# MiniMax-AI/VTP

Hardware: NVIDIA H100
Metric: images/sec (256x256 encode+decode+3-loss step) (higher is better)
Workload: dtype bf16

## Files before the change

vtp_b200/csrc/attention.cu:

```cuda
#include <stdlib.h>

#include "attention.h"
#include "host.h"
#include "ptx.cuh"

namespace vtp {

static constexpr int ATT_THREADS = 384;
static constexpr int MAX_PREFIX = ATT_MAX_PREFIX;
static constexpr int SQ = 0, SK = 16384, SV = SK + 32768, SBAR = SV + 32768;
static constexpr int SPCLS = SBAR + 128;
static constexpr int ATT_SMEM = SPCLS + 512 + 1024;

__device__ __forceinline__ float ex2f(float x) {
    float y;
    asm("ex2.approx.ftz.f32 %0, %1;" : "=f"(y) : "f"(x));
    return y;
}
__device__ __forceinline__ uint32_t sw128_off(int row, int col ) {
    return row * 128 + ((((col >> 3) ^ (row & 7)) << 4) | ((col & 7) << 1));
}

template <int NKT>
__global__ void __launch_bounds__(ATT_THREADS, 1) attn_fwd_kernel(const __grid_constant__ CUtensorMap tm, const AttnDev p) {
    constexpr int NK = 128 * NKT;
    extern __shared__ uint8_t smem_raw[];
    uint8_t* smem = reinterpret_cast<uint8_t*>((reinterpret_cast<uintptr_t>(smem_raw) + 1023) & ~uintptr_t(1023));
    uint64_t* bars = reinterpret_cast<uint64_t*>(smem + SBAR);
    uint64_t* bar_qk = bars + 0;
    uint64_t* bar_v = bars + 1;

    const int warp = threadIdx.x >> 5, lane = threadIdx.x & 31;
    const int qt = blockIdx.x, h = blockIdx.y, b = p.pack ? blockIdx.z * p.pack : blockIdx.z;
    const int D = p.D, T = p.T, prefix = p.prefix, HW = p.HW;
    const long seq_row0 = (long)b * T;
    const int kvrows = NK;

    if (threadIdx.x == 0) {
        tma_prefetch_desc(&tm);
        mbar_init(bar_qk, 1), mbar_init(bar_v, 1);
        fence_barrier_init();
    }
    __syncthreads();

    if (warp < 8) {
        setmaxnreg_inc<200>();
        const int wg = warp >> 2, tw = threadIdx.x & 127, c4 = lane & 3;
        int rr[2], qpos[2], qtok[2], pseq[2], kmin[2], kmax[2];
        bool row_valid[2];
#pragma unroll
        for (int i = 0; i < 2; ++i) {
            rr[i] = 64 * wg + 16 * (tw >> 5) + (lane >> 2) + 8 * i;
            qpos[i] = 128 * qt + rr[i];
            qtok[i] = prefix + qpos[i];
            pseq[i] = p.pack ? rr[i] / T : 0;
            row_valid[i] = p.pack ? (pseq[i] < p.pack && b + pseq[i] < p.B) : (qpos[i] < HW);
            kmin[i] = p.pack ? (row_valid[i] ? pseq[i] * T : 0) : 0;
            kmax[i] = p.pack ? (row_valid[i] ? kmin[i] + T : 0) : (p.causal ? min(HW, qpos[i] + 1) : HW);
        }
        mbar_wait(bar_qk, 0);
        float s[NK / 2];
        {
            const uint32_t qa = smem_u32(smem + SQ) + wg * 8192, ka = smem_u32(smem + SK);
            wgmma_fence();
#pragma unroll
            for (int j = 0; j < 4; ++j) {
                const uint64_t ad = wgmma_desc_sw128(qa + j * 32, 0, 1024), bd = wgmma_desc_sw128(ka + j * 32, 0, 1024);
                if constexpr (NKT == 2) wgmma_m64n256_ss<0, 0>(s, ad, bd, j > 0);
                else wgmma_m64n128_ss<0, 0>(s, ad, bd, j > 0);
            }
            wgmma_commit();
        }
        float s_pre[2][MAX_PREFIX];
#pragma unroll
        for (int j = 0; j < MAX_PREFIX; ++j) {
            float acc0 = 0.f, acc1 = 0.f;
            if (j < prefix) {
                const uint4* kp = reinterpret_cast<const uint4*>(p.qkv + (seq_row0 + j) * 3 * D + D + h * 64 + 16 * c4);
#pragma unroll
                for (int c = 0; c < 2; ++c) {
                    const uint4 w = __ldg(kp + c);
                    const uint4 q0 = *reinterpret_cast<const uint4*>(smem + SQ + sw128_off(rr[0], 16 * c4 + 8 * c));
                    const uint4 q1 = *reinterpret_cast<const uint4*>(smem + SQ + sw128_off(rr[1], 16 * c4 + 8 * c));
                    const uint32_t kw[4] = {w.x, w.y, w.z, w.w}, qw0[4] = {q0.x, q0.y, q0.z, q0.w}, qw1[4] = {q1.x, q1.y, q1.z, q1.w};
#pragma unroll
                    for (int e = 0; e < 4; ++e) {
                        acc0 += bf16_lo(qw0[e]) * bf16_lo(kw[e]) + bf16_hi(qw0[e]) * bf16_hi(kw[e]);
                        acc1 += bf16_lo(qw1[e]) * bf16_lo(kw[e]) + bf16_hi(qw1[e]) * bf16_hi(kw[e]);
                    }
                }
            }
            acc0 += __shfl_xor_sync(0xffffffffu, acc0, 1), acc1 += __shfl_xor_sync(0xffffffffu, acc1, 1);
            acc0 += __shfl_xor_sync(0xffffffffu, acc0, 2), acc1 += __shfl_xor_sync(0xffffffffu, acc1, 2);
            s_pre[0][j] = (j < prefix && (!p.causal || j <= qtok[0])) ? acc0 : -INFINITY;
            s_pre[1][j] = (j < prefix && (!p.causal || j <= qtok[1])) ? acc1 : -INFINITY;
        }
        wgmma_wait<0>();
        fence_regs(s);
        float m[2], msc[2], l[2];
#pragma unroll
        for (int i = 0; i < 2; ++i) {
            m[i] = -INFINITY;
#pragma unroll
            for (int j = 0; j < MAX_PREFIX; ++j) m[i] = fmaxf(m[i], s_pre[i][j]);
        }
#pragma unroll
        for (int jn = 0; jn < NK / 8; ++jn)
#pragma unroll
            for (int i = 0; i < 2; ++i)
#pragma unroll
                for (int c = 0; c < 2; ++c) {
                    const int key = 8 * jn + 2 * c4 + c;
                    if (key >= kmin[i] && key < kmax[i]) m[i] = fmaxf(m[i], s[4 * jn + 2 * i + c]);
                }
        float p_pre[2][MAX_PREFIX];
#pragma unroll
        for (int i = 0; i < 2; ++i) {
            m[i] = fmaxf(m[i], __shfl_xor_sync(0xffffffffu, m[i], 1));
            m[i] = fmaxf(m[i], __shfl_xor_sync(0xffffffffu, m[i], 2));
            msc[i] = (m[i] == -INFINITY) ? 0.f : m[i] * p.scale_log2;
            l[i] = 0.f;
#pragma unroll
            for (int j = 0; j < MAX_PREFIX; ++j) {
                p_pre[i][j] = (s_pre[i][j] == -INFINITY) ? 0.f : ex2f(s_pre[i][j] * p.scale_log2 - msc[i]);
                if (c4 == 0) l[i] += p_pre[i][j];
                p_pre[i][j] = bf16_round(p_pre[i][j]);
            }
        }
#pragma unroll
        for (int jn = 0; jn < NK / 8; ++jn)
#pragma unroll
            for (int i = 0; i < 2; ++i)
#pragma unroll
                for (int c = 0; c < 2; ++c) {
                    const int key = 8 * jn + 2 * c4 + c;
                    float& v = s[4 * jn + 2 * i + c];
                    v = (key >= kmin[i] && key < kmax[i]) ? ex2f(v * p.scale_log2 - msc[i]) : 0.f;
                    l[i] += v;
                }
        mbar_wait(bar_v, 0);
        float o[32];
        {
            const uint32_t va = smem_u32(smem + SV);
            wgmma_fence();
#pragma unroll
            for (int kk = 0; kk < NK / 16; ++kk) {
                const uint32_t a[4] = {pack_bf16x2(s[8 * kk], s[8 * kk + 1]), pack_bf16x2(s[8 * kk + 2], s[8 * kk + 3]),
                                       pack_bf16x2(s[8 * kk + 4], s[8 * kk + 5]), pack_bf16x2(s[8 * kk + 6], s[8 * kk + 7])};
                wgmma_m64n64_rs<1>(o, a, wgmma_desc_sw128(va + kk * 2048, 8192, 1024), kk > 0);
            }
            wgmma_commit();
            wgmma_wait<0>();
            fence_regs(o);
        }
#pragma unroll
        for (int i = 0; i < 2; ++i) {
            l[i] += __shfl_xor_sync(0xffffffffu, l[i], 1);
            l[i] += __shfl_xor_sync(0xffffffffu, l[i], 2);
        }
#pragma unroll
        for (int j = 0; j < MAX_PREFIX; ++j) {
            if (j < prefix) {
                const __nv_bfloat16* vp = p.qkv + (seq_row0 + j) * 3 * D + 2 * D + h * 64 + 2 * c4;
#pragma unroll
                for (int jn = 0; jn < 8; ++jn) {
                    const uint32_t w = __ldg(reinterpret_cast<const uint32_t*>(vp + 8 * jn));
#pragma unroll
                    for (int i = 0; i < 2; ++i)
                        o[4 * jn + 2 * i] += p_pre[i][j] * bf16_lo(w), o[4 * jn + 2 * i + 1] += p_pre[i][j] * bf16_hi(w);
                }
            }
        }
#pragma unroll
        for (int i = 0; i < 2; ++i) {
            if (!row_valid[i]) continue;
            const float inv = 1.f / l[i];
            __nv_bfloat16* op = p.out + (seq_row0 + qtok[i]) * D + h * 64 + 2 * c4;
#pragma unroll
            for (int jn = 0; jn < 8; ++jn)
                *reinterpret_cast<uint32_t*>(op + 8 * jn) = pack_bf16x2(o[4 * jn + 2 * i] * inv, o[4 * jn + 2 * i + 1] * inv);
            if (p.lse && c4 == 0) {
                if (p.pack) p.lse[((long)(b + pseq[i]) * p.H + h) * T + (rr[i] - pseq[i] * T)] = m[i] * p.scale + logf(l[i]);
                else p.lse[((long)b * p.H + h) * T + qtok[i]] = m[i] * p.scale + logf(l[i]);
            }
        }
    } else {
        setmaxnreg_dec<104>();
        if (warp != 8) return;
        if (lane == 0) {
            const int row_q = (int)seq_row0 + prefix + 128 * qt;
            const int row_k = (int)seq_row0 + prefix;
            mbar_expect_tx(bar_qk, 16384 + 16384 * NKT);
            tma_load_2d(smem + SQ, &tm, bar_qk, h * 64, row_q);
            for (int i = 0; i < NKT; ++i) tma_load_2d(smem + SK + i * 16384, &tm, bar_qk, D + h * 64, row_k + 128 * i);
            mbar_expect_tx(bar_v, 16384 * NKT);
            for (int i = 0; i < NKT; ++i) tma_load_2d(smem + SV + i * 16384, &tm, bar_v, 2 * D + h * 64, row_k + 128 * i);
        }
        if (qt == 0 && prefix > 0) {
            mbar_wait(bar_qk, 0);
            mbar_wait(bar_v, 0);
            for (int j = 0; j < prefix; ++j) {
                float qf[64];
                {
                    const uint4* qp = reinterpret_cast<const uint4*>(p.qkv + (seq_row0 + j) * 3 * D + h * 64);
#pragma unroll
                    for (int c = 0; c < 8; ++c) {
                        const uint4 w = __ldg(qp + c);
                        qf[c * 8 + 0] = bf16_lo(w.x), qf[c * 8 + 1] = bf16_hi(w.x), qf[c * 8 + 2] = bf16_lo(w.y);
                        qf[c * 8 + 3] = bf16_hi(w.y), qf[c * 8 + 4] = bf16_lo(w.z), qf[c * 8 + 5] = bf16_hi(w.z);
                        qf[c * 8 + 6] = bf16_lo(w.w), qf[c * 8 + 7] = bf16_hi(w.w);
                    }
                }
                auto dot_row = [&](const uint4* kp, bool from_smem, int row) {
                    float acc = 0.f;
#pragma unroll
                    for (int c = 0; c < 8; ++c) {
                        const uint4 w = from_smem ? *reinterpret_cast<const uint4*>(smem + SK + sw128_off(row, c * 8))
                                                  : __ldg(kp + c);
                        acc += qf[c * 8 + 0] * bf16_lo(w.x) + qf[c * 8 + 1] * bf16_hi(w.x) + qf[c * 8 + 2] * bf16_lo(w.y) +
                               qf[c * 8 + 3] * bf16_hi(w.y) + qf[c * 8 + 4] * bf16_lo(w.z) + qf[c * 8 + 5] * bf16_hi(w.z) +
                               qf[c * 8 + 6] * bf16_lo(w.w) + qf[c * 8 + 7] * bf16_hi(w.w);
                    }
                    return acc;
                };
                float sp[MAX_PREFIX], s[8];
                float m = -INFINITY;
#pragma unroll
                for (int t = 0; t < MAX_PREFIX; ++t) {
                    sp[t] = -INFINITY;
                    if (t < prefix && (!p.causal || t <= j))
                        sp[t] = dot_row(reinterpret_cast<const uint4*>(p.qkv + (seq_row0 + t) * 3 * D + D + h * 64), false, 0);
                    m = fmaxf(m, sp[t]);
                }
#pragma unroll
                for (int i = 0; i < 8; ++i) {
                    const int kk = lane + 32 * i;
                    s[i] = -INFINITY;
                    if (kk < HW && kk < kvrows && (!p.causal || prefix + kk <= j)) s[i] = dot_row(nullptr, true, kk);
                    m = fmaxf(m, s[i]);
                }
                m = warp_max(m);
                const float msc = m * p.scale_log2;
                float l = 0.f;
                __nv_bfloat16* pcls = reinterpret_cast<__nv_bfloat16*>(smem + SPCLS);
                __syncwarp();
#pragma unroll
                for (int i = 0; i < 8; ++i) {
                    const float e = (s[i] == -INFINITY) ? 0.f : ex2f(s[i] * p.scale_log2 - msc);
                    l += e;
                    pcls[lane + 32 * i] = __float2bfloat16_rn(e);
                }
                l = warp_sum(l);
                __syncwarp();
                float a0 = 0.f, a1 = 0.f, c0 = 0.f, c1 = 0.f;
#pragma unroll
                for (int t = 0; t < MAX_PREFIX; ++t) {
                    if (t < prefix && sp[t] != -INFINITY) {
                        const float pe = ex2f(sp[t] * p.scale_log2 - msc);
                        l += pe;
                        const uint32_t w = __ldg(reinterpret_cast<const uint32_t*>(p.qkv + (seq_row0 + t) * 3 * D + 2 * D + h * 64) + lane);
                        a0 += bf16_round(pe) * bf16_lo(w), a1 += bf16_round(pe) * bf16_hi(w);
                    }
                }
                const int kend = min(HW, kvrows);
                for (int k8 = 0; k8 < kend; k8 += 8) {
                    const uint4 pw = *reinterpret_cast<const uint4*>(pcls + k8);
                    const uint32_t pr[4] = {pw.x, pw.y, pw.z, pw.w};
#pragma unroll
                    for (int u = 0; u < 8; ++u) {
                        const float pk = (u & 1) ? bf16_hi(pr[u >> 1]) : bf16_lo(pr[u >> 1]);
                        const uint32_t w = *reinterpret_cast<const uint32_t*>(smem + SV + sw128_off(k8 + u, 2 * lane));
                        if (u & 1) c0 += pk * bf16_lo(w), c1 += pk * bf16_hi(w);
                        else a0 += pk * bf16_lo(w), a1 += pk * bf16_hi(w);
                    }
                }
                a0 += c0, a1 += c1;
                const float inv = 1.f / l;
                *reinterpret_cast<uint32_t*>(p.out + (seq_row0 + j) * D + h * 64 + 2 * lane) = pack_bf16x2(a0 * inv, a1 * inv);
                if (p.lse && lane == 0) p.lse[((long)b * p.H + h) * T + j] = m * p.scale + logf(l);
            }
        }
    }
}


__global__ void attn_fwd_f32_kernel(const float* __restrict__ qkv, float* __restrict__ out, int T, int H, int causal,
                                    float scale) {
    extern __shared__ float sm[];
    const int D = H * 64, h = blockIdx.x, b = blockIdx.y;
    float* Ks = sm;
    float* Vs = Ks + (long)T * 65;
    float* Ps = Vs + (long)T * 64;
    const float* base = qkv + (long)b * T * 3 * D;
    for (int i = threadIdx.x; i < T * 64; i += blockDim.x) {
        const int t = i >> 6, d = i & 63;
        Ks[t * 65 + d] = base[(long)t * 3 * D + D + h * 64 + d];
        Vs[t * 64 + d] = base[(long)t * 3 * D + 2 * D + h * 64 + d];
    }
    __syncthreads();
    const int warp = threadIdx.x >> 5, lane = threadIdx.x & 31, nw = blockDim.x >> 5;
    float* pw = Ps + (long)warp * T;
    for (int q = warp; q < T; q += nw) {
        const float* qp = base + (long)q * 3 * D + h * 64;
        float qf[64];
#pragma unroll
        for (int d = 0; d < 64; ++d) qf[d] = qp[d];
        const int kend = causal ? q + 1 : T;
        float m = -INFINITY;
        for (int k = lane; k < kend; k += 32) {
            float acc = 0.f;
#pragma unroll
            for (int d = 0; d < 64; ++d) acc += qf[d] * Ks[k * 65 + d];
            acc *= scale;
            pw[k] = acc;
            m = fmaxf(m, acc);
        }
        m = warp_max(m);
        float l = 0.f;
        for (int k = lane; k < kend; k += 32) {
            const float e = expf(pw[k] - m);
            pw[k] = e;
            l += e;
        }
        l = warp_sum(l);
        __syncwarp();
        float a0 = 0.f, a1 = 0.f;
        for (int k = 0; k < kend; ++k) {
            const float pk = pw[k];
            a0 += pk * Vs[k * 64 + lane], a1 += pk * Vs[k * 64 + 32 + lane];
        }
        float* op = out + ((long)b * T + q) * D + h * 64;
        op[lane] = a0 / l, op[32 + lane] = a1 / l;
        __syncwarp();
    }
}

}

using namespace vtp;

extern "C" int vtp_attention_fwd(const void* qkv, void* out, float* lse, int B, int T, int H, int prefix, int causal,
                                 vtp_stream_t st) {
    VTP_CHECK_ARG(qkv && out && B > 0 && T > 0 && H > 0, "attention_fwd: bad args");
    VTP_CHECK_ARG(prefix >= 0 && prefix <= MAX_PREFIX && prefix < T, "attention_fwd: prefix must be in [0,%d]", MAX_PREFIX);
    const int HW = T - prefix;
    VTP_CHECK_ARG(HW <= 256 || !causal, "attention_fwd: causal attention over %d > 256 non-prefix tokens is not supported",
                  HW);
    VTP_CHECK_ARG(B <= 65535 && H <= 65535, "attention_fwd: grid too large");
    const int D = H * 64;
    AttnDev p;
    p.qkv = (const __nv_bfloat16*)qkv, p.out = (__nv_bfloat16*)out, p.lse = lse;
    p.B = B, p.T = T, p.H = H, p.D = D, p.prefix = prefix, p.HW = HW, p.causal = causal;
    p.nkt = HW > 128 ? 2 : 1;
    p.scale = 0.125f;
    p.scale_log2 = 0.125f * 1.4426950408889634f;
    p.pack = 0;
    if (!causal && T <= 64 && B > 1 && getenv("VTP_ATTN_NO_PACK") == nullptr) {
        p.pack = 128 / T;
        p.prefix = 0, p.HW = T, p.nkt = 1;
    }
    CUtensorMap tm;
    uint64_t dims[2] = {(uint64_t)3 * D, (uint64_t)B * T}, strides[1] = {(uint64_t)3 * D * 2};
    uint32_t box[2] = {64, 128};
    int rc = make_tmap_bf16(&tm, qkv, 2, dims, strides, box);
    if (rc) return rc;
    if (HW > 256) return attn_fwd_long(tm, p, (cudaStream_t)st);
    static bool configured = false;
    if (!configured) {
        VTP_CUDA(cudaFuncSetAttribute(attn_fwd_kernel<1>, cudaFuncAttributeMaxDynamicSharedMemorySize, ATT_SMEM));
        VTP_CUDA(cudaFuncSetAttribute(attn_fwd_kernel<2>, cudaFuncAttributeMaxDynamicSharedMemorySize, ATT_SMEM));
        configured = true;
    }
    dim3 grid(p.pack ? 1 : ceil_div(HW, 128), H, p.pack ? ceil_div(B, p.pack) : B);
    if (p.nkt == 2) attn_fwd_kernel<2><<<grid, ATT_THREADS, ATT_SMEM, (cudaStream_t)st>>>(tm, p);
    else attn_fwd_kernel<1><<<grid, ATT_THREADS, ATT_SMEM, (cudaStream_t)st>>>(tm, p);
    VTP_LAUNCH_CHECK();
    return VTP_OK;
}

extern "C" int vtp_attention_fwd_f32(const float* qkv, float* out, int B, int T, int H, int causal, vtp_stream_t st) {
    VTP_CHECK_ARG(qkv && out && B > 0 && T > 0 && H > 0 && B <= 65535, "attention_fwd_f32: bad args");
    const int nw = 8;
    const size_t smem = ((size_t)T * 65 + (size_t)T * 64 + (size_t)nw * T) * sizeof(float);
    if (smem > 220 * 1024) {
        VTP_CHECK_ARG(!causal, "attention_fwd_f32: causal attention over T=%d (beyond the smem-resident kernel) is not "
                               "supported", T);
        return attn_fwd_f32_tiled(qkv, out, B, T, H, (cudaStream_t)st);
    }
    static size_t configured = 0;
    if (smem > configured) {
        VTP_CUDA(cudaFuncSetAttribute(attn_fwd_f32_kernel, cudaFuncAttributeMaxDynamicSharedMemorySize, (int)smem));
        configured = smem;
    }
    attn_fwd_f32_kernel<<<dim3(H, B), nw * 32, smem, (cudaStream_t)st>>>(qkv, out, T, H, causal, 0.125f);
    VTP_LAUNCH_CHECK();
    return VTP_OK;
}
```

Measured before the change: 704.4.

## Make short-sequence attention forward persistent with double-buffered TMA and parallel prefix warps

Result: faster. 719.0, median of 6 (+2.1%).

```diff
diff --git a/vtp_b200/csrc/attention.cu b/vtp_b200/csrc/attention.cu
--- a/vtp_b200/csrc/attention.cu
+++ b/vtp_b200/csrc/attention.cu
@@ -8,9 +8,17 @@
 
 static constexpr int ATT_THREADS = 384;
 static constexpr int MAX_PREFIX = ATT_MAX_PREFIX;
-static constexpr int SQ = 0, SK = 16384, SV = SK + 32768, SBAR = SV + 32768;
-static constexpr int SPCLS = SBAR + 128;
-static constexpr int ATT_SMEM = SPCLS + 512 + 1024;
+static constexpr int PREFIX_WARPS = 3;
+static constexpr int CONSUMER_REGS = 200, WG2_REGS = 104;
+template <int NKT>
+struct FwdSmem {
+    static constexpr int TILE = 16384 * NKT;
+    static constexpr int SLOT = 3 * TILE;
+    static constexpr int BAR = 2 * SLOT;
+    static constexpr int PCLS = BAR + 64;
+    static constexpr int QCLS = PCLS + PREFIX_WARPS * 512;
+    static constexpr int BYTES = QCLS + PREFIX_WARPS * 128 + 1024;
+};
 
 __device__ __forceinline__ float ex2f(float x) {
     float y;
@@ -21,268 +29,300 @@
     return row * 128 + ((((col >> 3) ^ (row & 7)) << 4) | ((col & 7) << 1));
 }
 
+template <int NKT, bool DENSE>
+__device__ __forceinline__ void fwd_block(const AttnDev& p, const uint8_t* sl, int blk, int h, int b, long seq_row0) {
+    constexpr int NK = 128 * NKT;
+    constexpr int TILE = FwdSmem<NKT>::TILE;
+    const int lane = threadIdx.x & 31, tw = threadIdx.x & 127, c4 = lane & 3;
+    const int D = p.D, T = p.T, prefix = p.prefix, HW = p.HW;
+    int rr[2], qtok[2], pseq[2], kmin[2], kmax[2];
+    bool row_valid[2];
+#pragma unroll
+    for (int i = 0; i < 2; ++i) {
+        rr[i] = 64 * blk + 16 * (tw >> 5) + (lane >> 2) + 8 * i;
+        qtok[i] = prefix + rr[i];
+        pseq[i] = p.pack ? rr[i] / T : 0;
+        row_valid[i] = p.pack ? (pseq[i] < p.pack && b + pseq[i] < p.B) : (rr[i] < HW);
+        kmin[i] = p.pack ? (row_valid[i] ? pseq[i] * T : 0) : 0;
+        kmax[i] = p.pack ? (row_valid[i] ? kmin[i] + T : 0) : (p.causal ? min(HW, rr[i] + 1) : HW);
+    }
+    float s[NK / 2];
+    {
+        const uint32_t qa = smem_u32(sl) + blk * 8192, ka = smem_u32(sl + TILE);
+        wgmma_fence();
+#pragma unroll
+        for (int j = 0; j < 4; ++j) {
+            const uint64_t ad = wgmma_desc_sw128(qa + j * 32, 0, 1024), bd = wgmma_desc_sw128(ka + j * 32, 0, 1024);
+            if constexpr (NKT == 2) wgmma_m64n256_ss<0, 0>(s, ad, bd, j > 0);
+            else wgmma_m64n128_ss<0, 0>(s, ad, bd, j > 0);
+        }
+        wgmma_commit();
+    }
+    float s_pre[2][MAX_PREFIX];
+#pragma unroll
+    for (int j = 0; j < MAX_PREFIX; ++j) {
+        float acc0 = 0.f, acc1 = 0.f;
+        if (j < prefix) {
+            const uint4* kp = reinterpret_cast<const uint4*>(p.qkv + (seq_row0 + j) * 3 * D + D + h * 64 + 16 * c4);
+#pragma unroll
+            for (int c = 0; c < 2; ++c) {
+                const uint4 w = __ldg(kp + c);
+                const uint4 q0 = *reinterpret_cast<const uint4*>(sl + sw128_off(rr[0], 16 * c4 + 8 * c));
+                const uint4 q1 = *reinterpret_cast<const uint4*>(sl + sw128_off(rr[1], 16 * c4 + 8 * c));
+                const uint32_t kw[4] = {w.x, w.y, w.z, w.w}, qw0[4] = {q0.x, q0.y, q0.z, q0.w}, qw1[4] = {q1.x, q1.y, q1.z, q1.w};
+#pragma unroll
+                for (int e = 0; e < 4; ++e) {
+                    acc0 += bf16_lo(qw0[e]) * bf16_lo(kw[e]) + bf16_hi(qw0[e]) * bf16_hi(kw[e]);
+                    acc1 += bf16_lo(qw1[e]) * bf16_lo(kw[e]) + bf16_hi(qw1[e]) * bf16_hi(kw[e]);
+                }
+            }
+        }
+        acc0 += __shfl_xor_sync(0xffffffffu, acc0, 1), acc1 += __shfl_xor_sync(0xffffffffu, acc1, 1);
+        acc0 += __shfl_xor_sync(0xffffffffu, acc0, 2), acc1 += __shfl_xor_sync(0xffffffffu, acc1, 2);
+        s_pre[0][j] = (j < prefix && (!p.causal || j <= qtok[0])) ? acc0 : -INFINITY;
+        s_pre[1][j] = (j < prefix && (!p.causal || j <= qtok[1])) ? acc1 : -INFINITY;
+    }
+    wgmma_wait<0>();
+    fence_regs(s);
+    float m[2], msc[2], l[2];
+#pragma unroll
+    for (int i = 0; i < 2; ++i) {
+        m[i] = -INFINITY;
+#pragma unroll
+        for (int j = 0; j < MAX_PREFIX; ++j) m[i] = fmaxf(m[i], s_pre[i][j]);
+    }
+#pragma unroll
+    for (int jn = 0; jn < NK / 8; ++jn)
+#pragma unroll
+        for (int i = 0; i < 2; ++i)
+#pragma unroll
+            for (int c = 0; c < 2; ++c) {
+                const int key = 8 * jn + 2 * c4 + c;
+                if (DENSE || (key >= kmin[i] && key < kmax[i])) m[i] = fmaxf(m[i], s[4 * jn + 2 * i + c]);
+            }
+    float p_pre[2][MAX_PREFIX];
+#pragma unroll
+    for (int i = 0; i < 2; ++i) {
+        m[i] = fmaxf(m[i], __shfl_xor_sync(0xffffffffu, m[i], 1));
+        m[i] = fmaxf(m[i], __shfl_xor_sync(0xffffffffu, m[i], 2));
+        msc[i] = (m[i] == -INFINITY) ? 0.f : m[i] * p.scale_log2;
+        l[i] = 0.f;
+#pragma unroll
+        for (int j = 0; j < MAX_PREFIX; ++j) {
+            p_pre[i][j] = (s_pre[i][j] == -INFINITY) ? 0.f : ex2f(s_pre[i][j] * p.scale_log2 - msc[i]);
+            if (c4 == 0) l[i] += p_pre[i][j];
+            p_pre[i][j] = bf16_round(p_pre[i][j]);
+        }
+    }
+    uint32_t a[NK / 4];
+#pragma unroll
+    for (int jn = 0; jn < NK / 8; ++jn) {
+        float v[4];
+#pragma unroll
+        for (int i = 0; i < 2; ++i)
+#pragma unroll
+            for (int c = 0; c < 2; ++c) {
+                const int key = 8 * jn + 2 * c4 + c;
+                const float x = s[4 * jn + 2 * i + c];
+                v[2 * i + c] = (DENSE || (key >= kmin[i] && key < kmax[i])) ? ex2f(x * p.scale_log2 - msc[i]) : 0.f;
+                l[i] += v[2 * i + c];
+            }
+        a[2 * jn] = pack_bf16x2(v[0], v[1]), a[2 * jn + 1] = pack_bf16x2(v[2], v[3]);
+    }
+    float o[32];
+    {
+        const uint32_t va = smem_u32(sl + 2 * TILE);
+        wgmma_fence();
+#pragma unroll
+        for (int kk = 0; kk < NK / 16; ++kk) {
+            const uint32_t ak[4] = {a[4 * kk], a[4 * kk + 1], a[4 * kk + 2], a[4 * kk + 3]};
+            wgmma_m64n64_rs<1>(o, ak, wgmma_desc_sw128(va + kk * 2048, 8192, 1024), kk > 0);
+        }
+        wgmma_commit();
+        wgmma_wait<0>();
+        fence_regs(o);
+    }
+#pragma unroll
+    for (int i = 0; i < 2; ++i) {
+        l[i] += __shfl_xor_sync(0xffffffffu, l[i], 1);
+        l[i] += __shfl_xor_sync(0xffffffffu, l[i], 2);
+    }
+#pragma unroll
+    for (int j = 0; j < MAX_PREFIX; ++j) {
+        if (j < prefix) {
+            const __nv_bfloat16* vp = p.qkv + (seq_row0 + j) * 3 * D + 2 * D + h * 64 + 2 * c4;
+#pragma unroll
+            for (int jn = 0; jn < 8; ++jn) {
+                const uint32_t w = __ldg(reinterpret_cast<const uint32_t*>(vp + 8 * jn));
+#pragma unroll
+                for (int i = 0; i < 2; ++i)
+                    o[4 * jn + 2 * i] += p_pre[i][j] * bf16_lo(w), o[4 * jn + 2 * i + 1] += p_pre[i][j] * bf16_hi(w);
+            }
+        }
+    }
+#pragma unroll
+    for (int i = 0; i < 2; ++i) {
+        if (!row_valid[i]) continue;
+        const float inv = 1.f / l[i];
+        __nv_bfloat16* op = p.out + (seq_row0 + qtok[i]) * D + h * 64 + 2 * c4;
+#pragma unroll
+        for (int jn = 0; jn < 8; ++jn)
+            *reinterpret_cast<uint32_t*>(op + 8 * jn) = pack_bf16x2(o[4 * jn + 2 * i] * inv, o[4 * jn + 2 * i + 1] * inv);
+        if (p.lse && c4 == 0) {
+            if (p.pack) p.lse[((long)(b + pseq[i]) * p.H + h) * T + (rr[i] - pseq[i] * T)] = m[i] * p.scale + logf(l[i]);
+            else p.lse[((long)b * p.H + h) * T + qtok[i]] = m[i] * p.scale + logf(l[i]);
+        }
+    }
+}
+
 template <int NKT>
-__global__ void __launch_bounds__(ATT_THREADS, 1) attn_fwd_kernel(const __grid_constant__ CUtensorMap tm, const AttnDev p) {
+__device__ __forceinline__ void fwd_prefix_row(const AttnDev& p, const uint8_t* sl, uint4* qs, __nv_bfloat16* pcls, int j,
+                                               int h, int b, long seq_row0) {
     constexpr int NK = 128 * NKT;
+    constexpr int TILE = FwdSmem<NKT>::TILE;
+    const int lane = threadIdx.x & 31;
+    const int D = p.D, T = p.T, prefix = p.prefix, HW = p.HW;
+    const uint8_t* sk = sl + TILE;
+    const uint8_t* sv = sl + 2 * TILE;
+    __syncwarp();
+    if (lane < 8) qs[lane] = __ldg(reinterpret_cast<const uint4*>(p.qkv + (seq_row0 + j) * 3 * D + h * 64) + lane);
+    __syncwarp();
+    auto dot_row = [&](const uint4* kp, bool from_smem, int row) {
+        float acc = 0.f;
+#pragma unroll 1
+        for (int c = 0; c < 8; ++c) {
+            const uint4 w = from_smem ? *reinterpret_cast<const uint4*>(sk + sw128_off(row, c * 8)) : __ldg(kp + c);
+            const uint4 q = qs[c];
+            acc += bf16_lo(q.x) * bf16_lo(w.x) + bf16_hi(q.x) * bf16_hi(w.x) + bf16_lo(q.y) * bf16_lo(w.y) +
+                   bf16_hi(q.y) * bf16_hi(w.y) + bf16_lo(q.z) * bf16_lo(w.z) + bf16_hi(q.z) * bf16_hi(w.z) +
+                   bf16_lo(q.w) * bf16_lo(w.w) + bf16_hi(q.w) * bf16_hi(w.w);
+        }
+        return acc;
+    };
+    float sp[MAX_PREFIX], s[8];
+    float m = -INFINITY;
+#pragma unroll
+    for (int t = 0; t < MAX_PREFIX; ++t) {
+        sp[t] = -INFINITY;
+        if (t < prefix && (!p.causal || t <= j))
+            sp[t] = dot_row(reinterpret_cast<const uint4*>(p.qkv + (seq_row0 + t) * 3 * D + D + h * 64), false, 0);
+        m = fmaxf(m, sp[t]);
+    }
+#pragma unroll
+    for (int i = 0; i < 8; ++i) {
+        const int kk = lane + 32 * i;
+        s[i] = -INFINITY;
+        if (kk < HW && kk < NK && (!p.causal || prefix + kk <= j)) s[i] = dot_row(nullptr, true, kk);
+        m = fmaxf(m, s[i]);
+    }
+    m = warp_max(m);
+    const float msc = m * p.scale_log2;
+    float l = 0.f;
+    __syncwarp();
+#pragma unroll
+    for (int i = 0; i < 8; ++i) {
+        const float e = (s[i] == -INFINITY) ? 0.f : ex2f(s[i] * p.scale_log2 - msc);
+        l += e;
+        pcls[lane + 32 * i] = __float2bfloat16_rn(e);
+    }
+    l = warp_sum(l);
+    __syncwarp();
+    float a0 = 0.f, a1 = 0.f, c0 = 0.f, c1 = 0.f;
+#pragma unroll
+    for (int t = 0; t < MAX_PREFIX; ++t) {
+        if (t < prefix && sp[t] != -INFINITY) {
+            const float pe = ex2f(sp[t] * p.scale_log2 - msc);
+            l += pe;
+            const uint32_t w = __ldg(reinterpret_cast<const uint32_t*>(p.qkv + (seq_row0 + t) * 3 * D + 2 * D + h * 64) + lane);
+            a0 += bf16_round(pe) * bf16_lo(w), a1 += bf16_round(pe) * bf16_hi(w);
+        }
+    }
+    const int kend = min(HW, NK);
+    for (int k8 = 0; k8 < kend; k8 += 8) {
+        const uint4 pw = *reinterpret_cast<const uint4*>(pcls + k8);
+        const uint32_t pr[4] = {pw.x, pw.y, pw.z, pw.w};
+#pragma unroll
+        for (int u = 0; u < 8; ++u) {
+            const float pk = (u & 1) ? bf16_hi(pr[u >> 1]) : bf16_lo(pr[u >> 1]);
+            const uint32_t w = *reinterpret_cast<const uint32_t*>(sv + sw128_off(k8 + u, 2 * lane));
+            if (u & 1) c0 += pk * bf16_lo(w), c1 += pk * bf16_hi(w);
+            else a0 += pk * bf16_lo(w), a1 += pk * bf16_hi(w);
+        }
+    }
+    a0 += c0, a1 += c1;
+    const float inv = 1.f / l;
+    *reinterpret_cast<uint32_t*>(p.out + (seq_row0 + j) * D + h * 64 + 2 * lane) = pack_bf16x2(a0 * inv, a1 * inv);
+    if (p.lse && lane == 0) p.lse[((long)b * p.H + h) * T + j] = m * p.scale + logf(l);
+}
+
+template <int NKT, bool DENSE>
+__global__ void __launch_bounds__(ATT_THREADS, 1)
+    attn_fwd_persistent_kernel(const __grid_constant__ CUtensorMap tm, const AttnDev p) {
+    using L = FwdSmem<NKT>;
     extern __shared__ uint8_t smem_raw[];
     uint8_t* smem = reinterpret_cast<uint8_t*>((reinterpret_cast<uintptr_t>(smem_raw) + 1023) & ~uintptr_t(1023));
-    uint64_t* bars = reinterpret_cast<uint64_t*>(smem + SBAR);
-    uint64_t* bar_qk = bars + 0;
-    uint64_t* bar_v = bars + 1;
+    uint64_t* full = reinterpret_cast<uint64_t*>(smem + L::BAR);
+    uint64_t* empty = full + 2;
 
     const int warp = threadIdx.x >> 5, lane = threadIdx.x & 31;
-    const int qt = blockIdx.x, h = blockIdx.y, b = p.pack ? blockIdx.z * p.pack : blockIdx.z;
-    const int D = p.D, T = p.T, prefix = p.prefix, HW = p.HW;
-    const long seq_row0 = (long)b * T;
-    const int kvrows = NK;
+    const int H = p.H, T = p.T, prefix = p.prefix;
+    const int items = (p.pack ? (p.B + p.pack - 1) / p.pack : p.B) * H;
+    const int prefix_warps = min(prefix, PREFIX_WARPS);
 
     if (threadIdx.x == 0) {
         tma_prefetch_desc(&tm);
-        mbar_init(bar_qk, 1), mbar_init(bar_v, 1);
+        for (int s = 0; s < 2; ++s) mbar_init(full + s, 1), mbar_init(empty + s, 8 + prefix_warps);
         fence_barrier_init();
     }
     __syncthreads();
 
     if (warp < 8) {
-        setmaxnreg_inc<200>();
-        const int wg = warp >> 2, tw = threadIdx.x & 127, c4 = lane & 3;
-        int rr[2], qpos[2], qtok[2], pseq[2], kmin[2], kmax[2];
-        bool row_valid[2];
-#pragma unroll
-        for (int i = 0; i < 2; ++i) {
-            rr[i] = 64 * wg + 16 * (tw >> 5) + (lane >> 2) + 8 * i;
-            qpos[i] = 128 * qt + rr[i];
-            qtok[i] = prefix + qpos[i];
-            pseq[i] = p.pack ? rr[i] / T : 0;
-            row_valid[i] = p.pack ? (pseq[i] < p.pack && b + pseq[i] < p.B) : (qpos[i] < HW);
-            kmin[i] = p.pack ? (row_valid[i] ? pseq[i] * T : 0) : 0;
-            kmax[i] = p.pack ? (row_valid[i] ? kmin[i] + T : 0) : (p.causal ? min(HW, qpos[i] + 1) : HW);
-        }
-        mbar_wait(bar_qk, 0);
-        float s[NK / 2];
-        {
-            const uint32_t qa = smem_u32(smem + SQ) + wg * 8192, ka = smem_u32(smem + SK);
-            wgmma_fence();
-#pragma unroll
-            for (int j = 0; j < 4; ++j) {
-                const uint64_t ad = wgmma_desc_sw128(qa + j * 32, 0, 1024), bd = wgmma_desc_sw128(ka + j * 32, 0, 1024);
-                if constexpr (NKT == 2) wgmma_m64n256_ss<0, 0>(s, ad, bd, j > 0);
-                else wgmma_m64n128_ss<0, 0>(s, ad, bd, j > 0);
-            }
-            wgmma_commit();
-        }
-        float s_pre[2][MAX_PREFIX];
-#pragma unroll
-        for (int j = 0; j < MAX_PREFIX; ++j) {
-            float acc0 = 0.f, acc1 = 0.f;
-            if (j < prefix) {
-                const uint4* kp = reinterpret_cast<const uint4*>(p.qkv + (seq_row0 + j) * 3 * D + D + h * 64 + 16 * c4);
-#pragma unroll
-                for (int c = 0; c < 2; ++c) {
-                    const uint4 w = __ldg(kp + c);
-                    const uint4 q0 = *reinterpret_cast<const uint4*>(smem + SQ + sw128_off(rr[0], 16 * c4 + 8 * c));
-                    const uint4 q1 = *reinterpret_cast<const uint4*>(smem + SQ + sw128_off(rr[1], 16 * c4 + 8 * c));
-                    const uint32_t kw[4] = {w.x, w.y, w.z, w.w}, qw0[4] = {q0.x, q0.y, q0.z, q0.w}, qw1[4] = {q1.x, q1.y, q1.z, q1.w};
-#pragma unroll
-                    for (int e = 0; e < 4; ++e) {
-                        acc0 += bf16_lo(qw0[e]) * bf16_lo(kw[e]) + bf16_hi(qw0[e]) * bf16_hi(kw[e]);
-                        acc1 += bf16_lo(qw1[e]) * bf16_lo(kw[e]) + bf16_hi(qw1[e]) * bf16_hi(kw[e]);
-                    }
+        setmaxnreg_inc<CONSUMER_REGS>();
+        const int wg = __shfl_sync(0xffffffffu, warp >> 2, 0);
+        int it = 0;
+        for (int item = blockIdx.x; item < items; item += gridDim.x, ++it) {
+            const int slot = it & 1, h = item % H, sq = item / H;
+            const int b = p.pack ? sq * p.pack : sq;
+            const int nrows = p.pack ? min(p.pack, p.B - b) * T : p.HW;
+            const uint8_t* sl = smem + slot * L::SLOT;
+            mbar_wait(full + slot, (it >> 1) & 1);
+#pragma unroll 1
+            for (int blk = wg; 64 * blk < nrows; blk += 2) fwd_block<NKT, DENSE>(p, sl, blk, h, b, (long)b * T);
+            __syncwarp();
+            if (lane == 0) mbar_arrive(empty + slot);
+        }
+    } else {
+        setmaxnreg_dec<WG2_REGS>();
+        if (warp == 8) {
+            if (lane != 0) return;
+            int it = 0;
+            for (int item = blockIdx.x; item < items; item += gridDim.x, ++it) {
+                const int slot = it & 1, h = item % H, sq = item / H;
+                const int row0 = (p.pack ? sq * p.pack : sq) * T + prefix;
+                uint8_t* sl = smem + slot * L::SLOT;
+                if (it >= 2) mbar_wait(empty + slot, ((it >> 1) - 1) & 1);
+                mbar_expect_tx(full + slot, 3 * L::TILE);
+                for (int i = 0; i < NKT; ++i) {
+                    tma_load_2d(sl + i * 16384, &tm, full + slot, h * 64, row0 + 128 * i);
+                    tma_load_2d(sl + L::TILE + i * 16384, &tm, full + slot, p.D + h * 64, row0 + 128 * i);
+                    tma_load_2d(sl + 2 * L::TILE + i * 16384, &tm, full + slot, 2 * p.D + h * 64, row0 + 128 * i);
                 }
             }
-            acc0 += __shfl_xor_sync(0xffffffffu, acc0, 1), acc1 += __shfl_xor_sync(0xffffffffu, acc1, 1);
-            acc0 += __shfl_xor_sync(0xffffffffu, acc0, 2), acc1 += __shfl_xor_sync(0xffffffffu, acc1, 2);
-            s_pre[0][j] = (j < prefix && (!p.causal || j <= qtok[0])) ? acc0 : -INFINITY;
-            s_pre[1][j] = (j < prefix && (!p.causal || j <= qtok[1])) ? acc1 : -INFINITY;
-        }
-        wgmma_wait<0>();
-        fence_regs(s);
-        float m[2], msc[2], l[2];
-#pragma unroll
-        for (int i = 0; i < 2; ++i) {
-            m[i] = -INFINITY;
-#pragma unroll
-            for (int j = 0; j < MAX_PREFIX; ++j) m[i] = fmaxf(m[i], s_pre[i][j]);
-        }
-#pragma unroll
-        for (int jn = 0; jn < NK / 8; ++jn)
-#pragma unroll
-            for (int i = 0; i < 2; ++i)
-#pragma unroll
-                for (int c = 0; c < 2; ++c) {
-                    const int key = 8 * jn + 2 * c4 + c;
-                    if (key >= kmin[i] && key < kmax[i]) m[i] = fmaxf(m[i], s[4 * jn + 2 * i + c]);
-                }
-        float p_pre[2][MAX_PREFIX];
-#pragma unroll
-        for (int i = 0; i < 2; ++i) {
-            m[i] = fmaxf(m[i], __shfl_xor_sync(0xffffffffu, m[i], 1));
-            m[i] = fmaxf(m[i], __shfl_xor_sync(0xffffffffu, m[i], 2));
-            msc[i] = (m[i] == -INFINITY) ? 0.f : m[i] * p.scale_log2;
-            l[i] = 0.f;
-#pragma unroll
-            for (int j = 0; j < MAX_PREFIX; ++j) {
-                p_pre[i][j] = (s_pre[i][j] == -INFINITY) ? 0.f : ex2f(s_pre[i][j] * p.scale_log2 - msc[i]);
-                if (c4 == 0) l[i] += p_pre[i][j];
-                p_pre[i][j] = bf16_round(p_pre[i][j]);
-            }
-        }
-#pragma unroll
-        for (int jn = 0; jn < NK / 8; ++jn)
-#pragma unroll
-            for (int i = 0; i < 2; ++i)
-#pragma unroll
-                for (int c = 0; c < 2; ++c) {
-                    const int key = 8 * jn + 2 * c4 + c;
-                    float& v = s[4 * jn + 2 * i + c];
-                    v = (key >= kmin[i] && key < kmax[i]) ? ex2f(v * p.scale_log2 - msc[i]) : 0.f;
-                    l[i] += v;
-                }
-        mbar_wait(bar_v, 0);
-        float o[32];
-        {
-            const uint32_t va = smem_u32(smem + SV);
-            wgmma_fence();
-#pragma unroll
-            for (int kk = 0; kk < NK / 16; ++kk) {
-                const uint32_t a[4] = {pack_bf16x2(s[8 * kk], s[8 * kk + 1]), pack_bf16x2(s[8 * kk + 2], s[8 * kk + 3]),
-                                       pack_bf16x2(s[8 * kk + 4], s[8 * kk + 5]), pack_bf16x2(s[8 * kk + 6], s[8 * kk + 7])};
-                wgmma_m64n64_rs<1>(o, a, wgmma_desc_sw128(va + kk * 2048, 8192, 1024), kk > 0);
-            }
-            wgmma_commit();
-            wgmma_wait<0>();
-            fence_regs(o);
-        }
-#pragma unroll
-        for (int i = 0; i < 2; ++i) {
-            l[i] += __shfl_xor_sync(0xffffffffu, l[i], 1);
-            l[i] += __shfl_xor_sync(0xffffffffu, l[i], 2);
-        }
-#pragma unroll
-        for (int j = 0; j < MAX_PREFIX; ++j) {
-            if (j < prefix) {
-                const __nv_bfloat16* vp = p.qkv + (seq_row0 + j) * 3 * D + 2 * D + h * 64 + 2 * c4;
-#pragma unroll
-                for (int jn = 0; jn < 8; ++jn) {
-                    const uint32_t w = __ldg(reinterpret_cast<const uint32_t*>(vp + 8 * jn));
-#pragma unroll
-                    for (int i = 0; i < 2; ++i)
-                        o[4 * jn + 2 * i] += p_pre[i][j] * bf16_lo(w), o[4 * jn + 2 * i + 1] += p_pre[i][j] * bf16_hi(w);
-                }
-            }
-        }
-#pragma unroll
-        for (int i = 0; i < 2; ++i) {
-            if (!row_valid[i]) continue;
-            const float inv = 1.f / l[i];
-            __nv_bfloat16* op = p.out + (seq_row0 + qtok[i]) * D + h * 64 + 2 * c4;
-#pragma unroll
-            for (int jn = 0; jn < 8; ++jn)
-                *reinterpret_cast<uint32_t*>(op + 8 * jn) = pack_bf16x2(o[4 * jn + 2 * i] * inv, o[4 * jn + 2 * i + 1] * inv);
-            if (p.lse && c4 == 0) {
-                if (p.pack) p.lse[((long)(b + pseq[i]) * p.H + h) * T + (rr[i] - pseq[i] * T)] = m[i] * p.scale + logf(l[i]);
-                else p.lse[((long)b * p.H + h) * T + qtok[i]] = m[i] * p.scale + logf(l[i]);
-            }
-        }
-    } else {
-        setmaxnreg_dec<104>();
-        if (warp != 8) return;
-        if (lane == 0) {
-            const int row_q = (int)seq_row0 + prefix + 128 * qt;
-            const int row_k = (int)seq_row0 + prefix;
-            mbar_expect_tx(bar_qk, 16384 + 16384 * NKT);
-            tma_load_2d(smem + SQ, &tm, bar_qk, h * 64, row_q);
-            for (int i = 0; i < NKT; ++i) tma_load_2d(smem + SK + i * 16384, &tm, bar_qk, D + h * 64, row_k + 128 * i);
-            mbar_expect_tx(bar_v, 16384 * NKT);
-            for (int i = 0; i < NKT; ++i) tma_load_2d(smem + SV + i * 16384, &tm, bar_v, 2 * D + h * 64, row_k + 128 * i);
-        }
-        if (qt == 0 && prefix > 0) {
-            mbar_wait(bar_qk, 0);
-            mbar_wait(bar_v, 0);
-            for (int j = 0; j < prefix; ++j) {
-                float qf[64];
-                {
-                    const uint4* qp = reinterpret_cast<const uint4*>(p.qkv + (seq_row0 + j) * 3 * D + h * 64);
-#pragma unroll
-                    for (int c = 0; c < 8; ++c) {
-                        const uint4 w = __ldg(qp + c);
-                        qf[c * 8 + 0] = bf16_lo(w.x), qf[c * 8 + 1] = bf16_hi(w.x), qf[c * 8 + 2] = bf16_lo(w.y);
-                        qf[c * 8 + 3] = bf16_hi(w.y), qf[c * 8 + 4] = bf16_lo(w.z), qf[c * 8 + 5] = bf16_hi(w.z);
-                        qf[c * 8 + 6] = bf16_lo(w.w), qf[c * 8 + 7] = bf16_hi(w.w);
-                    }
-                }
-                auto dot_row = [&](const uint4* kp, bool from_smem, int row) {
-                    float acc = 0.f;
-#pragma unroll
-                    for (int c = 0; c < 8; ++c) {
-                        const uint4 w = from_smem ? *reinterpret_cast<const uint4*>(smem + SK + sw128_off(row, c * 8))
-                                                  : __ldg(kp + c);
-                        acc += qf[c * 8 + 0] * bf16_lo(w.x) + qf[c * 8 + 1] * bf16_hi(w.x) + qf[c * 8 + 2] * bf16_lo(w.y) +
-                               qf[c * 8 + 3] * bf16_hi(w.y) + qf[c * 8 + 4] * bf16_lo(w.z) + qf[c * 8 + 5] * bf16_hi(w.z) +
-                               qf[c * 8 + 6] * bf16_lo(w.w) + qf[c * 8 + 7] * bf16_hi(w.w);
-                    }
-                    return acc;
-                };
-                float sp[MAX_PREFIX], s[8];
-                float m = -INFINITY;
-#pragma unroll
-                for (int t = 0; t < MAX_PREFIX; ++t) {
-                    sp[t] = -INFINITY;
-                    if (t < prefix && (!p.causal || t <= j))
-                        sp[t] = dot_row(reinterpret_cast<const uint4*>(p.qkv + (seq_row0 + t) * 3 * D + D + h * 64), false, 0);
-                    m = fmaxf(m, sp[t]);
-                }
-#pragma unroll
-                for (int i = 0; i < 8; ++i) {
-                    const int kk = lane + 32 * i;
-                    s[i] = -INFINITY;
-                    if (kk < HW && kk < kvrows && (!p.causal || prefix + kk <= j)) s[i] = dot_row(nullptr, true, kk);
-                    m = fmaxf(m, s[i]);
-                }
-                m = warp_max(m);
-                const float msc = m * p.scale_log2;
-                float l = 0.f;
-                __nv_bfloat16* pcls = reinterpret_cast<__nv_bfloat16*>(smem + SPCLS);
+        } else if (warp - 9 < prefix_warps) {
+            __nv_bfloat16* pcls = reinterpret_cast<__nv_bfloat16*>(smem + L::PCLS) + (warp - 9) * 256;
+            uint4* qs = reinterpret_cast<uint4*>(smem + L::QCLS) + (warp - 9) * 8;
+            int it = 0;
+            for (int item = blockIdx.x; item < items; item += gridDim.x, ++it) {
+                const int slot = it & 1, h = item % H, b = item / H;
+                mbar_wait(full + slot, (it >> 1) & 1);
+                for (int j = warp - 9; j < prefix; j += PREFIX_WARPS)
+                    fwd_prefix_row<NKT>(p, smem + slot * L::SLOT, qs, pcls, j, h, b, (long)b * T);
                 __syncwarp();
-#pragma unroll
-                for (int i = 0; i < 8; ++i) {
-                    const float e = (s[i] == -INFINITY) ? 0.f : ex2f(s[i] * p.scale_log2 - msc);
-                    l += e;
-                    pcls[lane + 32 * i] = __float2bfloat16_rn(e);
-                }
-                l = warp_sum(l);
-                __syncwarp();
-                float a0 = 0.f, a1 = 0.f, c0 = 0.f, c1 = 0.f;
-#pragma unroll
-                for (int t = 0; t < MAX_PREFIX; ++t) {
-                    if (t < prefix && sp[t] != -INFINITY) {
-                        const float pe = ex2f(sp[t] * p.scale_log2 - msc);
-                        l += pe;
-                        const uint32_t w = __ldg(reinterpret_cast<const uint32_t*>(p.qkv + (seq_row0 + t) * 3 * D + 2 * D + h * 64) + lane);
-                        a0 += bf16_round(pe) * bf16_lo(w), a1 += bf16_round(pe) * bf16_hi(w);
-                    }
-                }
-                const int kend = min(HW, kvrows);
-                for (int k8 = 0; k8 < kend; k8 += 8) {
-                    const uint4 pw = *reinterpret_cast<const uint4*>(pcls + k8);
-                    const uint32_t pr[4] = {pw.x, pw.y, pw.z, pw.w};
-#pragma unroll
-                    for (int u = 0; u < 8; ++u) {
-                        const float pk = (u & 1) ? bf16_hi(pr[u >> 1]) : bf16_lo(pr[u >> 1]);
-                        const uint32_t w = *reinterpret_cast<const uint32_t*>(smem + SV + sw128_off(k8 + u, 2 * lane));
-                        if (u & 1) c0 += pk * bf16_lo(w), c1 += pk * bf16_hi(w);
-                        else a0 += pk * bf16_lo(w), a1 += pk * bf16_hi(w);
-                    }
-                }
-                a0 += c0, a1 += c1;
-                const float inv = 1.f / l;
-                *reinterpret_cast<uint32_t*>(p.out + (seq_row0 + j) * D + h * 64 + 2 * lane) = pack_bf16x2(a0 * inv, a1 * inv);
-                if (p.lse && lane == 0) p.lse[((long)b * p.H + h) * T + j] = m * p.scale + logf(l);
-            }
-        }
-    }
-}
-
+                if (lane == 0) mbar_arrive(empty + slot);
+            }
+        }
+    }
+}
 
 __global__ void attn_fwd_f32_kernel(const float* __restrict__ qkv, float* __restrict__ out, int T, int H, int causal,
                                     float scale) {
@@ -367,13 +407,27 @@
     if (HW > 256) return attn_fwd_long(tm, p, (cudaStream_t)st);
     static bool configured = false;
     if (!configured) {
-        VTP_CUDA(cudaFuncSetAttribute(attn_fwd_kernel<1>, cudaFuncAttributeMaxDynamicSharedMemorySize, ATT_SMEM));
-        VTP_CUDA(cudaFuncSetAttribute(attn_fwd_kernel<2>, cudaFuncAttributeMaxDynamicSharedMemorySize, ATT_SMEM));
+        VTP_CUDA(cudaFuncSetAttribute(attn_fwd_persistent_kernel<1, false>, cudaFuncAttributeMaxDynamicSharedMemorySize,
+                                      FwdSmem<1>::BYTES));
+        VTP_CUDA(cudaFuncSetAttribute(attn_fwd_persistent_kernel<1, true>, cudaFuncAttributeMaxDynamicSharedMemorySize,
+                                      FwdSmem<1>::BYTES));
+        VTP_CUDA(cudaFuncSetAttribute(attn_fwd_persistent_kernel<2, false>, cudaFuncAttributeMaxDynamicSharedMemorySize,
+                                      FwdSmem<2>::BYTES));
+        VTP_CUDA(cudaFuncSetAttribute(attn_fwd_persistent_kernel<2, true>, cudaFuncAttributeMaxDynamicSharedMemorySize,
+                                      FwdSmem<2>::BYTES));
         configured = true;
     }
-    dim3 grid(p.pack ? 1 : ceil_div(HW, 128), H, p.pack ? ceil_div(B, p.pack) : B);
-    if (p.nkt == 2) attn_fwd_kernel<2><<<grid, ATT_THREADS, ATT_SMEM, (cudaStream_t)st>>>(tm, p);
-    else attn_fwd_kernel<1><<<grid, ATT_THREADS, ATT_SMEM, (cudaStream_t)st>>>(tm, p);
+    const int items = H * (p.pack ? ceil_div(B, p.pack) : B);
+    const int grid = items < num_sms() ? items : num_sms();
+    const bool dense = !p.pack && !causal && HW == 128 * p.nkt;
+    const cudaStream_t s = (cudaStream_t)st;
+    if (p.nkt == 2) {
+        if (dense) attn_fwd_persistent_kernel<2, true><<<grid, ATT_THREADS, FwdSmem<2>::BYTES, s>>>(tm, p);
+        else attn_fwd_persistent_kernel<2, false><<<grid, ATT_THREADS, FwdSmem<2>::BYTES, s>>>(tm, p);
+    } else {
+        if (dense) attn_fwd_persistent_kernel<1, true><<<grid, ATT_THREADS, FwdSmem<1>::BYTES, s>>>(tm, p);
+        else attn_fwd_persistent_kernel<1, false><<<grid, ATT_THREADS, FwdSmem<1>::BYTES, s>>>(tm, p);
+    }
     VTP_LAUNCH_CHECK();
     return VTP_OK;
 }
```
